# borgor/ripcurrents

Measured on AMD Instinct MI355X. Metric: frames/sec dense Farneback flow @1080p, higher is better.
Workload: dtype f32

## Files before the change

### ripcurrents_amd/csrc/flow_iter_kernels.hip

```cpp

#include <cstdlib>

#include "rc_device.h"

#define RC_ITER_BATCH 3
#define RC_RR_D 3

#ifdef RC_EXACT_BUILD
#define RC_FLOW_NS rc_flow_exact
#else
#define RC_FLOW_NS rc_flow_fast
#endif
namespace RC_FLOW_NS {

__device__ __forceinline__ float2 rc_flow_in(const RcIterArgs& a, const float2* fin, int gx, int gy) {
    if (a.in_mode == 0) return make_float2(0.f, 0.f);
    if (a.in_mode == 1) return fin[(size_t)gy * a.w + gx];
    float ax, ay;
    int sx = rc_src_x(gx, a.up_scale_x, a.fin_w, ax);
    int sx1 = min(sx + 1, a.fin_w - 1);
    int sy = rc_src_y(gy, a.up_scale_y, ay);
    int sy0 = rc_clampi(sy, 0, a.fin_h - 1), sy1 = rc_clampi(sy + 1, 0, a.fin_h - 1);
    const float2* S0 = fin + (size_t)sy0 * a.fin_w;
    const float2* S1 = fin + (size_t)sy1 * a.fin_w;
// ... 887 lines not shown
            p00[q] = S0[sx]; p01[q] = S0[sx1]; p10[q] = S1[sx]; p11[q] = S1[sx1];
        }
#pragma unroll
        for (int q = 0; q < NIT; q++) {
            float a0 = 1.f - ax, a1 = ax, b0 = 1.f - ay[q], b1 = ay[q];
            float r0x = p00[q].x * a0 + p01[q].x * a1, r1x = p10[q].x * a0 + p11[q].x * a1;
            float r0y = p00[q].y * a0 + p01[q].y * a1, r1y = p10[q].y * a0 + p11[q].y * a1;
            dx[q] = (r0x * b0 + r1x * b1) * a.up_mul;
            dy[q] = (r0y * b0 + r1y * b1) * a.up_mul;
        }
    }
}


__device__ __forceinline__ void rc_lds_barrier() { asm volatile("s_waitcnt lgkmcnt(0)\n\ts_barrier" ::: "memory"); }
__device__ __forceinline__ void rc_all_barrier() { asm volatile("s_waitcnt vmcnt(0) lgkmcnt(0)\n\ts_barrier" ::: "memory"); }

constexpr bool rc_recip_exact(int nt, int wp) {
    const unsigned r = (65536u + wp - 1) / wp;
    for (int t = 0; t < nt; t++)
        if ((int)((t * r) >> 16) != t / wp) return false;
    return true;
}

__device__ __forceinline__ void rc_glds16_s(const void* base, unsigned voff, uint32_t lds_wave_addr) {
    asm volatile("s_mov_b32 m0, %2\n\ts_nop 0\n\tglobal_load_lds_dwordx4 %0, %1" ::"v"(voff), "s"(base), "s"(lds_wave_addr) : "memory");
}
__device__ __forceinline__ void rc_glds4_s(const void* base, unsigned voff, uint32_t lds_wave_addr) {
    asm volatile("s_mov_b32 m0, %2\n\ts_nop 0\n\tglobal_load_lds_dword %0, %1" ::"v"(voff), "s"(base), "s"(lds_wave_addr) : "memory");
}

template <bool INTERIOR, int NT, int WP, int WN, int NWL>
__device__ __forceinline__ void rc_rrc_issue_window(const float4* __restrict__ RA1, const float* __restrict__ RB1,
                                                    uint32_t lds_a, uint32_t lds_b, int tid, int ox, int oy, int w, int h) {
    constexpr int QY = NT / WP, QX = NT % WP;
    const int wave_base = __builtin_amdgcn_readfirstlane(tid & ~63);
    static_assert(rc_recip_exact(NT, WP), "tid / WP by multiply and shift must be exact for every thread");
    int wy = (int)(__umul24((unsigned)tid, (65536u + WP - 1) / WP) >> 16), wx = tid - (int)__umul24((unsigned)wy, (unsigned)WP);
    int off = __mul24(oy + wy, w) + ox + wx;
#pragma unroll
    for (int q = 0; q < NWL; q++) {
        bool ok = (q + 1) * NT <= WN || tid + q * NT < WN;
        if (!INTERIOR) ok = ok && (unsigned)(ox + wx) < (unsigned)w && (unsigned)(oy + wy) < (unsigned)h;
        const unsigned p = ok ? (unsigned)off : 0u;
        if (q * NT + wave_base < WN) {
            rc_glds16_s(RA1, p << 4, lds_a + (uint32_t)(q * NT + wave_base) * 16u);
            rc_glds4_s(RB1, p << 2, lds_b + (uint32_t)(q * NT + wave_base) * 4u);
        }
        wx += QX; wy += QY; off += QY * w + QX;
        if (wx >= WP) { wx -= WP; wy += 1; off += w - WP; }
    }
}

template <bool INTERIOR, int NIT, int WW, int WH, int WP>
__device__ __forceinline__ void rc_rr_matrices(float (&m)[NIT][5], const float4 (&A0)[NIT], const float (&B0)[NIT],
                                               const float (&dx)[NIT], const float (&dy)[NIT], const float4* LA,
                                               const float* LB, int ox, int oy, const float4* __restrict__ RA1,
                                               const float* __restrict__ RB1, int gxo, const int (&gys)[NIT], int w, int h) {
    if constexpr (!INTERIOR) {
#pragma unroll
        for (int q = 0; q < NIT; q++) {
            RcGather g;
            rc_gather_window<WW, WH, WP>(g, LA, LB, ox, oy, RA1, RB1, gxo, gys[q], dx[q], dy[q], w, h);
            RcM5 v = rc_matrices_reg(A0[q], B0[q], g, dx[q], dy[q], gxo, gys[q], w, h, true);
            m[q][0] = v.m0; m[q][1] = v.m1; m[q][2] = v.m2; m[q][3] = v.m3; m[q][4] = v.m4;
        }
    } else {
        unsigned far = 0;
#pragma unroll
        for (int q = 0; q < NIT; q++) {
            RcGather g;
            const float fx = gxo + dx[q], fy = gys[q] + dy[q];
            const float flx = floorf(fx), fly = floorf(fy);
            const int x1 = (int)flx, y1 = (int)fly;
            g.fx = fx - flx;
            g.fy = fy - fly;
            g.inside = true;
            const int wx = x1 - ox, wy = y1 - oy;
            const bool in_win = (unsigned)wx < (unsigned)(WW - 1) && (unsigned)wy < (unsigned)(WH - 1);
            far |= in_win ? 0u : 1u << q;
            const unsigned i = in_win ? __umul24((unsigned)wy, (unsigned)WP) + (unsigned)wx : 0u;
            const float4* pa = (const float4*)((const char*)LA + (i << 4));
            const float* pb = (const float*)((const char*)LB + (i << 2));
            g.q00 = pa[0]; g.q01 = pa[1]; g.q10 = pa[WP]; g.q11 = pa[WP + 1];
            g.e00 = pb[0]; g.e01 = pb[1]; g.e10 = pb[WP]; g.e11 = pb[WP + 1];
            RcM5 v = rc_matrices_reg(A0[q], B0[q], g, dx[q], dy[q], gxo, gys[q], w, h, false);
            m[q][0] = v.m0; m[q][1] = v.m1; m[q][2] = v.m2; m[q][3] = v.m3; m[q][4] = v.m4;
        }
        if (__builtin_expect(far != 0, 0)) {
#pragma unroll
            for (int q = 0; q < NIT; q++) {
                if (far >> q & 1) {
                    RcGather g;
                    rc_gather_issue(g, RA1, RB1, gxo, gys[q], dx[q], dy[q], w, h);
                    RcM5 v = rc_matrices_reg(A0[q], B0[q], g, dx[q], dy[q], gxo, gys[q], w, h, false);
                    m[q][0] = v.m0; m[q][1] = v.m1; m[q][2] = v.m2; m[q][3] = v.m3; m[q][4] = v.m4;
                }
            }
        }
    }
}

template <bool INTERIOR, int IN_MODE, int GAUSS_, int NIT, int D, int MW, int NG>
__device__ __forceinline__ void rc_rrc_body(const RcIterArgs& a, const int zb, const int ze, float* smf, const uint32_t lds0, const int tx0, const int ty0) {
    constexpr int NT = NG * MW, MH = NG * NIT;
    constexpr int WW = MW + 2 * D, WH = MH + 2 * D, WP = WW, WN = WP * WH, NWL = (WN + NT - 1) / NT;
    constexpr int WNP = (WN + 63) & ~63;
    constexpr int MP = MW + 1, PLANE = MH * MP;
    static_assert(5 * PLANE <= 5 * WNP, "border-block M1 planes alias the R1 window");
    float4* LA = (float4*)smf;
    float* LB = smf + 4 * WNP;
    float* XR = LB + WNP;
    float* Ms = smf;
    const uint32_t lds_a = lds0, lds_b = lds0 + 16u * WNP;
    const int w = a.w, h = a.h;
    const int ox = tx0 - 2 - D, oy = ty0 - 2 - D;
#define RC_RRC_COORDS(tid_)                                                         \
    const int x = (tid_) & (MW - 1), grp = (tid_) / MW, ly0 = grp * NIT;            \
    const int px = tx0 - 2 + x;                                                     \
    const int gxo = INTERIOR ? px : rc_clampi(px, 0, w - 1);                        \
    int gys[NIT];                                                                   \
    _Pragma("unroll") for (int q = 0; q < NIT; q++)                                 \
        gys[q] = INTERIOR ? ty0 - 2 + ly0 + q : rc_clampi(ty0 - 2 + ly0 + q, 0, h - 1);

    float4 A0[NIT];
    float B0[NIT];
    float dx[NIT], dy[NIT];
    {
        const int tid = threadIdx.x;
        RC_RRC_COORDS(tid)
        const size_t s0 = (size_t)((a.slot0 + zb * a.zstep) % a.nslots) * a.R_slot_stride;
        const size_t s1 = (size_t)((a.slot1 + zb * a.zstep) % a.nslots) * a.R_slot_stride;
        rc_rrc_issue_window<INTERIOR, NT, WP, WN, NWL>(a.RA + s1, a.RB + s1, lds_a, lds_b, tid, ox, oy, w, h);
#pragma unroll
        for (int q = 0; q < NIT; q++) {
            const unsigned p0 = (unsigned)(gys[q] * w + gxo);
            A0[q] = (a.RA + s0)[p0];
            B0[q] = (a.RB + s0)[p0];
            rc_r0_prep(A0[q], B0[q]);
        }
        rc_rr_flow_in<IN_MODE, NIT, MW, MH, INTERIOR>(a, a.fin + (size_t)zb * a.fin_pair_stride, tx0, ty0, gxo, gys, dx, dy);
    }

    for (int z = zb; z < ze; z++) {
        const size_t s1 = (size_t)((a.slot1 + z * a.zstep) % a.nslots) * a.R_slot_stride;
        const float4* __restrict__ RA1 = a.RA + s1;
        const float* __restrict__ RB1 = a.RB + s1;
        const bool more = z + 1 < ze;
        int tid = threadIdx.x;
        asm volatile("" : "+v"(tid));
        RC_RRC_COORDS(tid)
        rc_all_barrier();

        float m[NIT][5];
        rc_rr_matrices<INTERIOR, NIT, WW, WH, WP>(m, A0, B0, dx, dy, LA, LB, ox, oy, RA1, RB1, gxo, gys, w, h);
        rc_rr_exchange<NIT, MW>(m, XR, grp, x);
        rc_lds_barrier();

        {
            float2 f1[NIT];
            rc_rr_flows<GAUSS_, NIT, MW, NG>(m, XR, grp, x, a.win, f1);
            float f1x[NIT], f1y[NIT];
#pragma unroll
            for (int q = 0; q < NIT; q++) { f1x[q] = f1[q].x; f1y[q] = f1[q].y; }
            rc_rr_matrices<INTERIOR, NIT, WW, WH, WP>(m, A0, B0, f1x, f1y, LA, LB, ox, oy, RA1, RB1, gxo, gys, w, h);
        }
        if (more) {
#pragma unroll
            for (int q = 0; q < NIT; q++) {
                const int i = (int)__umul24((unsigned)(gys[q] - oy), (unsigned)WP) + (gxo - ox);
                A0[q] = LA[i];
                B0[q] = LB[i];
                rc_r0_prep(A0[q], B0[q]);
            }
        }
        rc_lds_barrier();
        if constexpr (!INTERIOR) {
#pragma unroll
            for (int q = 0; q < NIT; q++)
#pragma unroll
                for (int c = 0; c < 5; c++) Ms[c * PLANE + (ly0 + q) * MP + x] = m[q][c];
            rc_lds_barrier();
#pragma unroll
            for (int q = 0; q < NIT; q++) {
                const int py = ty0 - 2 + ly0 + q;
                if ((unsigned)px >= (unsigned)w || (unsigned)py >= (unsigned)h) {
                    const int cx = gxo - (tx0 - 2), cy = gys[q] - (ty0 - 2);
#pragma unroll
                    for (int c = 0; c < 5; c++) m[q][c] = Ms[c * PLANE + cy * MP + cx];
                }
            }
        }
        rc_rr_exchange<NIT, MW>(m, XR, grp, x);
        rc_lds_barrier();

        if (more) {
            const size_t n1 = (size_t)((a.slot1 + (z + 1) * a.zstep) % a.nslots) * a.R_slot_stride;
            rc_rrc_issue_window<INTERIOR, NT, WP, WN, NWL>(a.RA + n1, a.RB + n1, lds_a, lds_b, tid, ox, oy, w, h);
        }

        {
            char* fout = a.fout + (size_t)z * a.fout_pair_stride;
            float2 f2[NIT];
            rc_rr_flows<GAUSS_, NIT, MW, NG>(m, XR, grp, x, a.win, f2);
            if (x >= 2 && x < MW - 2 && (INTERIOR || px < w)) {
                unsigned so = (unsigned)(ty0 - 2 + ly0) * (unsigned)a.fout_step + (unsigned)px * 8u;
#pragma unroll
                for (int q = 0; q < NIT; q++) {
                    const int ly = ly0 + q, py = ty0 - 2 + ly;
                    if (ly >= 2 && ly < MH - 2 && (INTERIOR || py < h)) *(float2*)(fout + so) = f2[q];
                    so += (unsigned)a.fout_step;
                }
            }
        }
        if (more) rc_rr_flow_in<IN_MODE, NIT, MW, MH, INTERIOR>(a, a.fin + (size_t)(z + 1) * a.fin_pair_stride, tx0, ty0, gxo, gys, dx, dy);
    }
#undef RC_RRC_COORDS
}

template <int IN_MODE, int GAUSS_, int NIT, int D, int MINB, int MW, int NG>
__global__ __launch_bounds__(NG * MW, MINB) void k_flow_iter2_rrc(RcIterArgs a, RcChainPlan cp) {
    constexpr int MH = NG * NIT, TW = MW - 4, TH = MH - 4;
    extern __shared__ __align__(16) float smf[];
    const int zb = cp.ngroups ? cp.start[blockIdx.y] : (int)blockIdx.y, ze = cp.ngroups ? cp.start[blockIdx.y + 1] : zb + 1;
    const int t = a.xcd_remap ? rc_xcd_remap(blockIdx.x, a.tiles_x * a.tiles_y) : (int)blockIdx.x;
    const int tx0 = (t % a.tiles_x) * TW, ty0 = (t / a.tiles_x) * TH;
    const bool interior = tx0 - 2 >= 5 && tx0 - 2 + MW <= a.w - 5 && ty0 - 2 >= 5 && ty0 - 2 + MH <= a.h - 5;
    const uint32_t lds0 = (uint32_t)(uintptr_t)(__attribute__((address_space(3))) void*)smf;
    if (interior) rc_rrc_body<true, IN_MODE, GAUSS_, NIT, D, MW, NG>(a, zb, ze, smf, lds0, tx0, ty0);
    else rc_rrc_body<false, IN_MODE, GAUSS_, NIT, D, MW, NG>(a, zb, ze, smf, lds0, tx0, ty0);
}

template <int IN_MODE, int G, int NIT, int D, int MINB, int MW = 32, int NG = 8>
static void launch_rrc_t(RcIterArgs a, const RcChainPlan& cp, int pairs, hipStream_t s) {
    constexpr int MH = NG * NIT, TW = MW - 4, TH = MH - 4;
    a.tw = TW; a.th = TH;
    a.tiles_x = (a.w + TW - 1) / TW; a.tiles_y = (a.h + TH - 1) / TH;
    constexpr int WN = (MW + 2 * D) * (MH + 2 * D), WNP = (WN + 63) & ~63;
    const size_t lds = sizeof(float) * (5 * WNP + NG * 2 * 5 * MW);
    RC_ALLOW_LDS((k_flow_iter2_rrc<IN_MODE, G, NIT, D, MINB, MW, NG>), lds);
    hipLaunchKernelGGL((k_flow_iter2_rrc<IN_MODE, G, NIT, D, MINB, MW, NG>), dim3(a.tiles_x * a.tiles_y, cp.ngroups ? cp.ngroups : pairs, 1), dim3(NG * MW), lds, s, a, cp);
}

static void rc_chain_plan(const RcIterArgs& a, int pairs, long long tiles, RcChainPlan& cp) {
    cp.ngroups = 0;
    const bool chainable = a.chain > 1 && pairs > 1 && (a.slot0 + a.zstep) % a.nslots == a.slot1 % a.nslots;
    if (!chainable) return;
    int chain = a.chain;
    if (!(a.ablate & RC_ABL_FORCE_CHAIN))
        while (chain > 1 && tiles * pairs / chain < (a.chain_min_blocks > 0 ? a.chain_min_blocks : 4096)) chain >>= 1;
    if (chain <= 1) return;
    int n = 0, z = 0;
    cp.start[0] = 0;
    while (z < pairs) {
        int left = pairs - z, c = left > chain ? chain : (left + 1) / 2;
        if (n == RC_MAX_CHAIN_GROUPS - 1) c = left;
        z += c;
        cp.start[++n] = z;
    }
    cp.ngroups = n;
}

template <int IN_MODE, int G>
static void launch_w3x2(RcIterArgs a, int pairs, hipStream_t s) {
    const long long tiles = (long long)((a.w + 27) / 28) * ((a.h + 27) / 28), blocks = tiles * pairs;
    RcChainPlan cp;
    rc_chain_plan(a, pairs, tiles, cp);
    if (cp.ngroups) launch_rrc_t<IN_MODE, G, 4, RC_RR_D, 4>(a, cp, pairs, s);
    else if (blocks < 512) launch_rrc_t<IN_MODE, G, 2, 4, 6>(a, cp, pairs, s);
    else if (blocks < 1024) launch_rrc_t<IN_MODE, G, 3, 4, 5>(a, cp, pairs, s);
    else launch_rrc_t<IN_MODE, G, 4, RC_RR_D, 4>(a, cp, pairs, s);
}

int rc_flow_iter_can_fuse2(const RcIterArgs& a) { return a.win.m == 1 && a.solve && a.addr32; }

int rc_flow_iter2_r0_reads(const RcIterArgs& a, int pairs) {
    RcChainPlan cp;
    rc_chain_plan(a, pairs, (long long)((a.w + 27) / 28) * ((a.h + 27) / 28), cp);
    return cp.ngroups ? cp.ngroups : pairs;
}

int rc_flow_chain_groups(const RcIterArgs& a, int pairs, int* starts, int cap) {
    RcChainPlan cp;
    rc_chain_plan(a, pairs, (long long)((a.w + 27) / 28) * ((a.h + 27) / 28), cp);
    for (int i = 0; i <= cp.ngroups && i < cap; i++) starts[i] = cp.start[i];
    return cp.ngroups;
}

void rc_launch_flow_iter2(const RcIterArgs& a, int pairs, hipStream_t s) {
    const int g = a.win.gaussian ? 1 : 0;
// ... 76 lines not shown
```

### ripcurrents_amd/csrc/rc_common.h

```cpp
#pragma once

#include <hip/hip_runtime.h>
#include <limits.h>
#include <stdint.h>

#include "../../include/rcflow.h"
#include "rc_plan.h"

#define RC_FMA(a, b, c) __builtin_fmaf((a), (b), (c))

__device__ __forceinline__ int rc_cvt_i32_x86(float v) {
    return (v >= -2147483648.f && v < 2147483648.f) ? (int)v : (int)0x80000000;
}

__device__ __forceinline__ const float2* rc_row2(const float* base, size_t step, int y) {
    return (const float2*)((const char*)base + (size_t)y * step);
}

__device__ __forceinline__ bool rc_sample_flow(const float* flow, size_t step, int w, int h, float x, float y,
                                               float& dx, float& dy) {
    int xind = rc_cvt_i32_x86(floorf(x)), yind = rc_cvt_i32_x86(floorf(y));
    float xrem = x - xind, yrem = y - yind;
    if (xind < 1 || yind < 1 || xind + 2 > w || yind + 2 > h) return false;
    const float2* r0 = rc_row2(flow, step, yind) + xind;
// ... 36 lines not shown
    const float* kern;
};

struct RcPolyArgs {
    const float* I;
    size_t I_slot_stride;
    const uint8_t* src8;
    size_t src8_step, src8_frame_stride;
    float4* RA;
    float* RB;
    size_t R_slot_stride;
    int slot0, nslots, zstep;
    int w, h;
    int tile_h;
    int valu_vertical;
    RcPolyK pk;
    int npyr;
    RcPyrFused py[2];
};

enum RcAblate : int {
    RC_ABL_EXACT_PLAIN_SCANS = 2,
    RC_ABL_EXACT_FUSED_M = 16,
    RC_ABL_PYR_STAGED = 4096,
    RC_ABL_TILE_WINDOW = 65536,
    RC_ABL_FORCE_SWEEP = 8388608,
    RC_ABL_FORCE_CHAIN = 33554432,
};

struct RcIterArgs {
    const float4* RA;
    const float* RB;
    size_t R_slot_stride;
    int slot0, slot1, nslots, zstep;
    int w, h;
    int in_mode;
    const float2* fin;
    size_t fin_pair_stride;
    int fin_w, fin_h;
    double up_scale_x, up_scale_y;
    float up_mul;
    int up_exact2;
    char* fout;
    size_t fout_step;
    size_t fout_pair_stride;
    int tw, th;
    int tiles_x, tiles_y;
    int solve;
    int xcd_remap;
    int ablate;
    int addr32;
    int chain_min_blocks;
    int chain;
    RcWindow win;
};

#define RC_MAX_CHAIN_GROUPS 64
struct RcChainPlan {
    int ngroups;
    int start[RC_MAX_CHAIN_GROUPS + 1];
};

struct RcExactArgs {
    const float4* RA;
    const float* RB;
    size_t n;
    int slot0, slot1, nslots, zstep;
    int w, h;
    const float2* fin;
    size_t fin_pair_stride;
    int fin_w, fin_h;
    double up_scale_x, up_scale_y;
    float up_mul;
    float2* flow;
    float* M;
    void* V;
    void* G;
    char* out;
    size_t out_step, out_pair_stride;
    int plain_scans;
    int fused_matrices;
    RcWindow win;
};
void rc_launch_exact_polyexp(const RcPolyArgs& a, int frames, hipStream_t s);
void rc_launch_exact_flow_init(const RcExactArgs& a, int pairs, hipStream_t s);
void rc_launch_exact_matrices(const RcExactArgs& a, int pairs, hipStream_t s);
void rc_launch_exact_window_solve(const RcExactArgs& a, int pairs, hipStream_t s);
int rc_exact_iteration_fused_ok(const RcExactArgs& a);
void rc_launch_exact_iteration_fused(const RcExactArgs& a, int pairs, hipStream_t s);

#define RC_MAX_DEVICES 64
#define RC_ALLOW_LDS(fn, lds)                                                                             \
    do {                                                                                                  \
        static size_t rc_seen_[RC_MAX_DEVICES] = {0};                                                     \
        int rc_dev_ = 0;                                                                                  \
        (void)hipGetDevice(&rc_dev_);                                                                     \
        if (rc_dev_ >= 0 && rc_dev_ < RC_MAX_DEVICES && (size_t)(lds) > rc_seen_[rc_dev_]) {             \
            (void)hipFuncSetAttribute((const void*)(fn), hipFuncAttributeMaxDynamicSharedMemorySize, (int)(lds)); \
            rc_seen_[rc_dev_] = (size_t)(lds);                                                            \
        }                                                                                                 \
    } while (0)

void rc_launch_pyr(const RcPyrArgs& a, int frames, size_t lds, hipStream_t s);
void rc_launch_polyexp(const RcPolyArgs& a, int frames, hipStream_t s);
int rc_polyexp_pyr_ok(const RcPolyArgs& a);
int rc_pyr_pair_ok(const RcPyrArgs& a1, const RcPyrArgs& a2);
// ... 32 lines not shown
```

### ripcurrents_amd/csrc/rc_host.h

```cpp
#pragma once

#include <initializer_list>
#include <string>
#include <vector>

#include "rc_common.h"

struct RcBuf {
    void* p = nullptr;
    size_t bytes = 0;
};

struct RcPlan {
    bool valid = false;
    int w = 0, h = 0;
    rc_farneback_params prm{};
    int nlev = 0;
    RcLevel lv[RC_MAX_LEVELS];
    size_t kern_off[RC_MAX_LEVELS];
    RcPolyK pk;
    RcWindow win;
    int nslots = 0, chunk = 0;
    int exact_taps = 0;
    int exact = 0;
// ... 180 lines not shown
    int ts_streak = 0;
    bool in_ts_push = false;
    RcPlan plan;
    RcBuf kern;
    RcBuf I[RC_MAX_LEVELS], RA[RC_MAX_LEVELS], RB[RC_MAX_LEVELS];
    RcBuf FA[RC_MAX_LEVELS], FB[RC_MAX_LEVELS];
    RcBuf stage_u8, stage_flow, stage_f32[4];
    RcBuf exM, exV, exG;
    void* pin[2] = {nullptr, nullptr};
    size_t pin_bytes = 0;
    hipEvent_t pin_free[2] = {nullptr, nullptr};
    int pin_i = 0;
    int pin_acq = -1, pin_w = 0, pin_h = 0;
    int flow_w = 0, flow_h = 0;
    int flow_fresh = 0;
    RcBuf lk;
    RcBuf fit_ws;
    RcBuf area_tab;
    RcBuf seed, seed_tab;
    int primed = 0, cur_slot = 0;
    int batch_primed = 0, batch_cur = 0;
    RcGraphCache batch_graph;
    RcGraphCache loop_graph;
    int loop_fc = 0;
    RcAnalysis an;
    RcTimex tx;
    RcFrameStab fs;
    RcRipMap rm;
    RcTracers tr;
    RcRegions rg;
    RcTracks tk;
    RcMotion mt;
    RcPhaseCorr pc;
};

struct RcProfRec {
    int id;
    hipEvent_t e0, e1;
    double bytes;
    double model_bytes;
};

struct rc_ctx {
    int device = 0;
    int max_w = 0, max_h = 0, nstreams = 0;
    RcSlot* slots = nullptr;
    int chunk = 32;
    int exact_taps = 0;
    int exact = -1;
    int fuse_iters = 1;
    int chain_min_blocks = 0;
    int chain = 8;
    int xcd_remap = 1;
    int poly_tile_h = 32;
    int frame_overlap = 1;
    int merge_small = 1;
    int overlap = 0;
    int poly_mfma = 0;
    int hist_blocks = 0;
    int fuse_pyr = 1;
    int ablate = 0;
    void* comm = nullptr;
    int prof_on = 0;
    std::vector<RcProfRec> prof_pending;
    std::vector<hipEvent_t> ev_pool;
    std::vector<int> prof_launches;
    std::vector<double> prof_ms, prof_bytes, prof_model_bytes;
};

#define RC_BUCKET_TABLE(X) \
    X(RC_B_FARNEBACK, "farneback") X(RC_B_POLAR, "polar") X(RC_B_THRESHOLD, "threshold") X(RC_B_OVERLAY, "overlay") \
    X(RC_B_EROSION, "erosion") X(RC_B_CODEC, "codec") X(RC_B_STREAM, "stream")
#define RC_KIND_TABLE(X) \
    X(RC_K_PYR, "pyr_level", RC_B_FARNEBACK) \
    X(RC_K_POLY, "polyexp", RC_B_FARNEBACK) \
    X(RC_K_ITER, "flow_iter", RC_B_FARNEBACK) \
    X(RC_K_HIST, "polar_hist", RC_B_THRESHOLD) \
    X(RC_K_THRESH, "thresholds", RC_B_THRESHOLD) \
    X(RC_K_CLASSIFY, "classify_accumulate", RC_B_THRESHOLD) \
    X(RC_K_ADVECT_FIELD, "advect_field", RC_B_STREAM) \
    X(RC_K_ADVECT_POINTS, "advect_points", RC_B_STREAM) \
    X(RC_K_POSTOP, "flow_postop", RC_B_FARNEBACK) \
    X(RC_K_COLOR, "flow_color", RC_B_THRESHOLD) \
    X(RC_K_ITER2, "flow_iter_x2", RC_B_FARNEBACK) \
    X(RC_K_PREPROC, "frame_preproc", RC_B_FARNEBACK) \
    X(RC_K_EDGES, "create_edges", RC_B_EROSION) \
    X(RC_K_DISPLAY, "streamline_display", RC_B_STREAM) \
    X(RC_K_HSV2BGR, "hsv_to_bgr", RC_B_THRESHOLD) \
    X(RC_K_OVERLAY, "create_output", RC_B_OVERLAY) \
    X(RC_K_FLOW_SEED, "flow_area_init", RC_B_FARNEBACK) \
    X(RC_K_TIMEX, "timex", RC_B_OVERLAY)  \
    X(RC_K_COLOR_U8, "frame_color", RC_B_OVERLAY)  \
    X(RC_K_FRAMESTAB, "framestab", RC_B_FARNEBACK)  \
    X(RC_K_RIPMAP, "ripmap", RC_B_FARNEBACK)  \
    X(RC_K_TRACKSTAB, "trackstab", RC_B_FARNEBACK)  \
    X(RC_K_TRACERS, "tracers", RC_B_STREAM)  \
    X(RC_K_REGIONS, "regions", RC_B_THRESHOLD)  \
    X(RC_K_TRACKS, "tracks", RC_B_THRESHOLD)  \
    X(RC_K_MOTION, "motion", RC_B_FARNEBACK)
#define RC_ROW_ID(id, ...) id,
enum { RC_BUCKET_TABLE(RC_ROW_ID) RC_B_BUCKETS };
enum { RC_KIND_TABLE(RC_ROW_ID) RC_K_KINDS };
enum { RC_K_LISTED = RC_K_MOTION };
static_assert(RC_K_LISTED == 25, "the rows before RC_K_MOTION keep their ids");
static_assert(RC_B_BUCKETS == RC_PROFILE_BUCKETS, "include/rcflow.h promises RC_PROFILE_BUCKETS buckets");

// ... 110 lines not shown
```

### ripcurrents_amd/csrc/rcflow_api.hip

```cpp

#include <cfloat>
#include <cmath>
#include <cstdarg>
#include <cstdio>
#include <cstring>

#include "rc_host.h"

static thread_local char g_err[512] = "";
void rc_set_error(const char* fmt, ...) {
    va_list ap;
    va_start(ap, fmt);
    vsnprintf(g_err, sizeof(g_err), fmt, ap);
    va_end(ap);
}
extern "C" const char* rcflow_last_error(void) { return g_err; }
extern "C" int rcflow_abi_version(void) { return RCFLOW_ABI_VERSION; }

int rc_buf_ensure(RcBuf& b, size_t bytes) {
    if (b.bytes >= bytes && b.p) return RC_OK;
    if (b.p) (void)hipFree(b.p);
    b.p = nullptr;
    b.bytes = 0;
    if (bytes == 0) return RC_OK;
// ... 276 lines not shown
    if (!s || !s->plan.valid || level < 0 || level >= s->plan.nlev || !d_flow) return RC_EINVAL;
    *d_flow = (float*)(which ? s->FB[level].p : s->FA[level].p);
    if (w) *w = s->plan.lv[level].w;
    if (h) *h = s->plan.lv[level].h;
    return *d_flow ? RC_OK : RC_ESTATE;
}

extern "C" int rcflow_debug_plan_poly(int n, double sigma, int exact_taps, float* g, float* xg, float* xxg, double* ig, int* n_eff,
                                      double* kdc) {
    if (n < 1 || n > RC_MAX_POLY_N || !(sigma >= 0) || !g || !xg || !xxg || !ig || !n_eff || !kdc) return RC_EINVAL;
    RcPolyK pk;
    const int rc = rc_plan_prepare_poly(n, sigma, exact_taps, pk);
    if (rc) return rc;
    memcpy(g, pk.g, (n + 1) * sizeof(float));
    memcpy(xg, pk.xg, (n + 1) * sizeof(float));
    memcpy(xxg, pk.xxg, (n + 1) * sizeof(float));
    ig[0] = pk.ig11; ig[1] = pk.ig03; ig[2] = pk.ig33; ig[3] = pk.ig55;
    *n_eff = pk.n_eff;
    *kdc = pk.kdc;
    return RC_OK;
}
extern "C" int rcflow_debug_plan_pyr_kernel(int ksize, double sigma, float* taps) {
    if (ksize < 1 || ksize > 1023 || !(sigma >= 0) || !taps) return RC_EINVAL;
    rc_plan_gaussian_kernel(ksize, sigma, taps);
    return RC_OK;
}
extern "C" int rcflow_debug_kind(int id, const char** name, const char** bucket) {
    if (id < 0 || id >= RC_K_LISTED || !name || !bucket) return RC_EINVAL;
    *name = kKindNames[id];
    *bucket = kBucketNames[kBucketOfKind[id]];
    return RC_OK;
}

extern "C" int rcflow_set_option(rc_ctx* ctx, const char* name, int value) {
    if (!ctx || !name) return RC_EINVAL;
    if (!strcmp(name, "chunk")) {
        if (value < 1 || value > 64) return RC_EINVAL;
        ctx->chunk = value;
    } else if (!strcmp(name, "exact_taps")) {
        ctx->exact_taps = value ? 1 : 0;
    } else if (!strcmp(name, "exact")) {
        if (value < -1 || value > 1) return RC_EINVAL;
        ctx->exact = value;
    } else if (!strcmp(name, "fuse_iters")) {
        ctx->fuse_iters = value ? 1 : 0;
    } else if (!strcmp(name, "chain")) {
        if (value < 1 || value > 64) return RC_EINVAL;
        ctx->chain = value;
    } else if (!strcmp(name, "chain_min_blocks")) {
        if (value < 0) return RC_EINVAL;
        ctx->chain_min_blocks = value;
    } else if (!strcmp(name, "xcd_remap")) {
        ctx->xcd_remap = value ? 1 : 0;
    } else if (!strcmp(name, "hist_blocks")) {
        if (value < 0 || value > 65535) return RC_EINVAL;
        ctx->hist_blocks = value;
    } else if (!strcmp(name, "overlap")) {
        ctx->overlap = value ? 1 : 0;
    } else if (!strcmp(name, "frame_overlap")) {
        if (value < 0 || value > 2) return RC_EINVAL;
        ctx->frame_overlap = value;
    } else if (!strcmp(name, "merge_small")) {
        ctx->merge_small = value ? 1 : 0;
    } else if (!strcmp(name, "poly_mfma")) {
        ctx->poly_mfma = value ? 1 : 0;
    } else if (!strcmp(name, "poly_tile_h")) {
        if (value != 32 && value != 48) return RC_EINVAL;
        ctx->poly_tile_h = value;
    } else if (!strcmp(name, "fuse_pyr")) {
        ctx->fuse_pyr = value != 0;
    } else if (!strcmp(name, "ablate")) {
        ctx->ablate = value;
    } else {
        rc_set_error("unknown option %s", name);
        return RC_EINVAL;
    }
    for (int i = 0; i < ctx->nstreams; i++) ctx->slots[i].plan.valid = false;
    return RC_OK;
}

extern "C" int rcflow_level_geometry(int w, int h, double pyr_scale, int levels, int k, int* wk, int* hk) {
    if (w <= 0 || h <= 0 || !(pyr_scale > 0 && pyr_scale < 1) || levels < 0 || k < 0) return RC_EINVAL;
    RcLevel L;
    rc_plan_level_geom(w, h, pyr_scale, k, L);
    if (wk) *wk = L.w;
    if (hk) *hk = L.h;
    return rc_plan_crop_levels(w, h, pyr_scale, levels);
}

static int ensure_plan(rc_ctx* ctx, RcSlot& s, int w, int h, const rc_farneback_params* p, int chunk, int nslots = 0) {
    if (nslots <= 0) nslots = chunk + 1;
    if (w <= 0 || h <= 0 || !rc_plan_params_valid(p)) {
        rc_set_error("invalid Farneback arguments (w=%d h=%d)", w, h);
        return RC_EINVAL;
    }
    if (w > ctx->max_w || h > ctx->max_h) {
        rc_set_error("frame %dx%d exceeds the context's %dx%d", w, h, ctx->max_w, ctx->max_h);
        return RC_ESIZE;
    }
    RcPlan& pl = s.plan;
    const rc_farneback_params& q = pl.prm;
    const bool same_prm = q.pyr_scale == p->pyr_scale && q.levels == p->levels && q.winsize == p->winsize &&
                          q.iterations == p->iterations && q.poly_n == p->poly_n && q.poly_sigma == p->poly_sigma &&
                          q.flags == p->flags;
    const int exact = ctx->exact >= 0 ? ctx->exact
                                      : (p->winsize / 2 == 0 || ((p->flags & RC_FARNEBACK_GAUSSIAN) && p->winsize / 2 <= 2));
    if (pl.valid && pl.w == w && pl.h == h && same_prm && pl.chunk == chunk &&
        pl.nslots == nslots && pl.exact_taps == ctx->exact_taps && pl.exact == exact)
        return RC_OK;
    rc_graph_drop(s.batch_graph);
    rc_graph_drop(s.loop_graph);
    RC_HIP(hipStreamSynchronize(s.cur));
    if (s.aux) RC_HIP(hipStreamSynchronize(s.aux));
    pl.valid = false;
    pl.w = w; pl.h = h; pl.chunk = chunk; pl.nslots = nslots;
    memset(&pl.prm, 0, sizeof(pl.prm));
    pl.prm.pyr_scale = p->pyr_scale; pl.prm.levels = p->levels; pl.prm.winsize = p->winsize;
    pl.prm.iterations = p->iterations; pl.prm.poly_n = p->poly_n; pl.prm.poly_sigma = p->poly_sigma;
    pl.prm.flags = p->flags;
    pl.exact_taps = ctx->exact_taps;
    pl.exact = exact;
    int L = rc_plan_crop_levels(w, h, p->pyr_scale, p->levels);
    pl.nlev = L + 1;
    size_t kern_total = 0;
    for (int k = 0; k <= L; k++) {
        rc_plan_level_geom(w, h, p->pyr_scale, k, pl.lv[k]);
        if (pl.lv[k].ksize > 1023) { rc_set_error("pyramid blur too wide"); return RC_EINVAL; }
        rc_plan_pick_pyr_tile(pl.lv[k], w, h);
        pl.kern_off[k] = kern_total;
        kern_total += (pl.lv[k].ksize + 3) & ~3;
    }
// ... 181 lines not shown
            a.fin = seeded; a.fin_pair_stride = a.n; a.fin_w = L.w; a.fin_h = L.h;
            a.up_scale_x = a.up_scale_y = 1.; a.up_mul = 1.f;
        }
        const double nb = (double)pairs * a.n;
        { RcProfScope ps(ctx, s.cur, RC_K_ITER, k, 8. * nb + (coarse ? 8. * pairs * cw * ch : seeded ? 8. * nb : 0.));
          rc_launch_exact_flow_init(a, pairs, s.cur); }
        for (int i = 0; i < iters; i++) {
            if (k == 0 && i == iters - 1) { a.out = (char*)d_out; a.out_step = out_step; a.out_pair_stride = out_pair_stride; }
            if (rc_exact_iteration_fused_ok(a)) {
                RcProfScope ps(ctx, s.cur, RC_K_ITER, k, 136. * nb);
                rc_launch_exact_iteration_fused(a, pairs, s.cur);
                continue;
            }
            { RcProfScope ps(ctx, s.cur, RC_K_ITER, k, 68. * nb); rc_launch_exact_matrices(a, pairs, s.cur); }
            { RcProfScope ps(ctx, s.cur, RC_K_ITER, k, (pl.win.gaussian ? 68. : 108.) * nb);
              rc_launch_exact_window_solve(a, pairs, s.cur); }
        }
        if (k == 0 && iters == 0)
            for (int z = 0; z < pairs; z++)
                RC_HIP(hipMemcpy2DAsync((char*)d_out + (size_t)z * out_pair_stride, out_step, a.flow + (size_t)z * a.n,
                                        (size_t)L.w * 8, (size_t)L.w * 8, (size_t)L.h, hipMemcpyDeviceToDevice, s.cur));
        coarse = a.flow;
        cw = L.w; ch = L.h;
    }
    RC_HIP(hipGetLastError());
    return RC_OK;
}

static int compute_flows(rc_ctx* ctx, RcSlot& s, int pairs, int slot0, float* d_out, size_t out_pair_stride,
                         size_t out_step, int slot1 = -1, int zstep = 1, const RcSeed* seed = nullptr) {
    if (!s.in_ts_push) s.ts_streak = 0;
    if (s.plan.exact && !s.plan.win.gaussian)
        return compute_flows_exact(ctx, s, pairs, slot0, d_out, out_pair_stride, out_step, slot1, zstep, seed);
    const bool exact = s.plan.exact != 0;
    RcPlan& pl = s.plan;
    const int iters = pl.prm.iterations;
    const float2* seeded = nullptr;
    if (seed) { int rc = launch_seed(ctx, s, pairs, *seed, &seeded); if (rc) return rc; }
    const float2* coarse = nullptr;
    int cw = 0, ch = 0;
    for (int k = pl.nlev - 1; k >= 0; k--) {
        const RcLevel& L = pl.lv[k];
        size_t n = (size_t)L.w * L.h;
        RcIterArgs a;
        memset(&a, 0, sizeof(a));
        a.RA = (const float4*)s.RA[k].p; a.RB = (const float*)s.RB[k].p; a.R_slot_stride = n;
        a.slot0 = slot0; a.slot1 = slot1 >= 0 ? slot1 : (slot0 + 1) % pl.nslots; a.nslots = pl.nslots; a.zstep = zstep;
        a.w = L.w; a.h = L.h;
        a.win = pl.win;
        a.xcd_remap = ctx->xcd_remap;
        a.ablate = ctx->ablate;
        a.chain = ctx->chain;
        a.chain_min_blocks = ctx->chain_min_blocks;
        const float2* cur_in = nullptr;
        int passes = iters > 0 ? iters : 1;
        int nout = 0;
        for (int i = 0; i < passes;) {
            double in_bytes;
            if (i == 0) {
                if (!coarse && seeded) { a.in_mode = 1; a.fin = seeded; a.fin_pair_stride = n; in_bytes = 8. * n; }
                else if (!coarse) { a.in_mode = 0; a.fin = nullptr; in_bytes = 0; }
                else {
                    a.in_mode = 2; a.fin = coarse; a.fin_pair_stride = (size_t)cw * ch;
                    a.fin_w = cw; a.fin_h = ch;
                    a.up_scale_x = 1. / ((double)L.w / cw);
                    a.up_scale_y = 1. / ((double)L.h / ch);
                    a.up_mul = (float)(1. / pl.prm.pyr_scale);
                    a.up_exact2 = (L.w == 2 * cw && L.h == 2 * ch) ? 1 : 0;
                    in_bytes = 8. * cw * ch;
                }
            } else {
                a.in_mode = 1; a.fin = cur_in; a.fin_pair_stride = n; in_bytes = 8. * n;
            }
            a.solve = iters > 0 ? 1 : 0;
            a.addr32 = n * 16 < (1ull << 32) && (size_t)L.h * (k == 0 ? (out_step > (size_t)L.w * 8 ? out_step : (size_t)L.w * 8) : (size_t)L.w * 8) < (1ull << 32);
            int fuse = (passes - i >= 2 && ctx->fuse_iters && rc_flow_fast::rc_flow_iter_can_fuse2(a)) ? 2 : 1;
            bool last = (i + fuse == passes);
            if (last && k == 0) {
                a.fout = (char*)d_out; a.fout_step = out_step; a.fout_pair_stride = out_pair_stride;
            } else {
                float2* dst = (float2*)((nout & 1) ? s.FB[k].p : s.FA[k].p);
                nout++;
                a.fout = (char*)dst; a.fout_step = (size_t)L.w * 8; a.fout_pair_stride = n * 8;
                cur_in = dst;
            }
            {
                double model = 0;
                if (i == 0) model += 60. * n + (coarse ? 8. * cw * ch : 0.);
                for (int j = i; j < i + fuse; j++) model += (j == passes - 1) ? 28. * n : 80. * n;
                const int r0 = fuse != 2 ? pairs : exact ? rc_flow_exact::rc_flow_iter2_r0_reads(a, pairs) : rc_flow_fast::rc_flow_iter2_r0_reads(a, pairs);
                RcProfScope ps(ctx, s.cur, fuse == 2 ? RC_K_ITER2 : RC_K_ITER, k,
                               (a.solve ? 20. * n * (pairs + r0) : 0.) + (double)pairs * (in_bytes + 8. * n), (double)pairs * model);
                if (exact) {
                    if (fuse == 2) rc_flow_exact::rc_launch_flow_iter2(a, pairs, s.cur);
                    else rc_flow_exact::rc_launch_flow_iter(a, pairs, s.cur);
                } else {
                    if (fuse == 2) rc_flow_fast::rc_launch_flow_iter2(a, pairs, s.cur);
                    else rc_flow_fast::rc_launch_flow_iter(a, pairs, s.cur);
                }
            }
            i += fuse;
        }
        coarse = cur_in;
        cw = L.w; ch = L.h;
    }
    RC_HIP(hipGetLastError());
// ... 362 lines not shown
    }
    cleanup();
    return rc;
}

void rc_graph_drop(RcGraphCache& g) {
    for (int i = 0; i < 2; i++) {
        if (g.exec[i]) (void)hipGraphExecDestroy((hipGraphExec_t)g.exec[i]);
        g.exec[i] = nullptr;
        g.eager[i] = 0;
    }
}

enum { RC_GRAPH_EAGER, RC_GRAPH_CAPTURE, RC_GRAPH_REPLAY };
static int graph_state(const RcGraphCache& g, int parity, const void* key, size_t key_bytes, bool allowed) {
    if (!allowed || memcmp(key, g.key[parity], key_bytes)) return RC_GRAPH_EAGER;
    return g.exec[parity] ? RC_GRAPH_REPLAY : g.eager[parity] ? RC_GRAPH_CAPTURE : RC_GRAPH_EAGER;
}

template <class Key, class Issue>
static int rc_graph_step(RcGraphCache& g, int parity, const Key& key, bool allowed, hipStream_t cap, hipStream_t run, Issue issue) {
    static_assert(sizeof(Key) <= sizeof(g.key[0]), "RcGraphCache::key too small");
    int rc;
    switch (graph_state(g, parity, &key, sizeof(key), allowed)) {
    case RC_GRAPH_REPLAY:
        RC_HIP(hipGraphLaunch((hipGraphExec_t)g.exec[parity], run));
        return RC_OK;
    case RC_GRAPH_CAPTURE: {
        hipGraph_t graph = nullptr;
        RC_HIP(hipStreamBeginCapture(cap, hipStreamCaptureModeRelaxed));
        rc = issue(cap);
        hipError_t e = hipStreamEndCapture(cap, &graph);
        if (rc) { if (graph) (void)hipGraphDestroy(graph); return rc; }
        if (e != hipSuccess || !graph) { rc_set_error("hipStreamEndCapture failed: %s", hipGetErrorString(e)); return RC_EHIP; }
        hipGraphExec_t exec = nullptr;
        e = hipGraphInstantiate(&exec, graph, nullptr, nullptr, 0);
        (void)hipGraphDestroy(graph);
        if (e != hipSuccess) { rc_set_error("hipGraphInstantiate failed: %s", hipGetErrorString(e)); return RC_EHIP; }
        g.exec[parity] = exec;
        RC_HIP(hipGraphLaunch(exec, run));
        return RC_OK;
    }
    default:
        if (g.exec[parity]) { (void)hipGraphExecDestroy((hipGraphExec_t)g.exec[parity]); g.exec[parity] = nullptr; }
        if ((rc = issue(run))) return rc;
        memcpy(g.key[parity], &key, sizeof(key));
        g.eager[parity] = 1;
        return RC_OK;
    }
}

struct RcLoopKey {
    rc_frame_loop loop;
    int w, h, pin, ring, ablate, chain;
    int seeded;
    void* hip_stream;
    void* d_frame; void* pin_host; void* d_flow;
};

static int loop_analysis(rc_ctx* ctx, RcSlot& s, int stream, const rc_frame_loop& L, int w, int h) {
    const size_t fs = (size_t)w * 8;
    float* d_flow = (float*)s.stage_flow.p;
    int rc;
    if ((rc = rc_loop_counter(ctx, s, false, 0))) return rc;
    if ((rc = rcflow_advect_field_dev(ctx, stream, d_flow, fs, w, h, L.dt, L.iterations, -1.f))) return rc;
    if (L.nseeds > 0 && (rc = rcflow_advect_points_dev(ctx, stream, L.d_seeds, L.nseeds, d_flow, fs, w, h, L.seed_dt, L.seed_iterations,
                                                       L.seed_upper, L.seed_variant, nullptr))) return rc;
    if ((rc = rcflow_histogram_dev(ctx, stream, d_flow, fs, w, h))) return rc;
    if ((rc = rcflow_thresholds_dev(ctx, stream))) return rc;
    if ((rc = rc_classify_accumulate(ctx, stream, d_flow, fs, w, h, -1, L.MID, L.LOWER, nullptr, 0, nullptr, 0, nullptr, 0,
                                     L.d_outmask, L.mask_step))) return rc;
    if (L.d_edges && (rc = rcflow_create_edges_dev(ctx, stream, L.d_outmask, L.mask_step, w, h, L.d_edges, L.edges_step))) return rc;
    return RC_OK;
}

static int loop_launches(rc_ctx* ctx, RcSlot& s, int stream, const rc_frame_loop& L, int pin, int w, int h, bool seeded) {
    const size_t fb = (size_t)w * h, fs = (size_t)w * 8;
    uint8_t* d_frame = (uint8_t*)s.stage_u8.p + (size_t)pin * fb;
    float* d_flow = (float*)s.stage_flow.p;
    const int cur = s.cur_slot, nxt = cur ^ 1;
    RC_HIP(hipMemcpyAsync(d_frame, s.pin[pin], fb, hipMemcpyHostToDevice, s.cur));
    int rc;
    if ((rc = expand_frames(ctx, s, d_frame, 0, w, 1, nxt))) return rc;
    const RcSeed seed = {d_flow, fs, 0};
    if ((rc = compute_flows(ctx, s, 1, cur, d_flow, 0, fs, nxt, 1, seeded ? &seed : nullptr))) return rc;
    return loop_analysis(ctx, s, stream, L, w, h);
}

extern "C" int rcflow_frame_loop_step(rc_ctx* ctx, int stream, const rc_farneback_params* p, const rc_frame_loop* loop) {
    RcSlot* s = rc_slot(ctx, stream);
    if (!s || !p || !loop) { if (s) rc_set_error("null argument"); return RC_EINVAL; }
    if (s->pin_acq < 0 || s->pin_acq != s->pin_i) { rc_set_error("no frame buffer acquired (rcflow_frame_buffer_acquire) since the last push"); return RC_ESTATE; }
    if (loop->nseeds < 0 || (loop->nseeds && !loop->d_seeds) || (loop->d_edges && !loop->d_outmask) || loop->iterations < 0) {
        rc_set_error("bad frame-loop configuration");
        return RC_EINVAL;
    }
    RC_HIP(hipSetDevice(ctx->device));
    const int w = s->pin_w, h = s->pin_h, pin = s->pin_acq;
    int rc;
    if (s->primed && s->an.w == w && s->an.h == h && (rc = rc_hist_book(*s, w, h, false))) return rc;
    if (!loop->use_graph) {
        if ((rc = rc_analysis_ensure(ctx, *s, w, h))) return rc;
        rc = push_staged_frame(ctx, s, pin, w, h, p);
        if (rc < 0) return rc;
        if (rc == 1) {
            s->loop_fc = 0;
            if ((rc = rc_loop_counter(ctx, *s, true, 0))) return rc;
            return 1;
        }
        if ((rc = loop_analysis(ctx, *s, stream, *loop, w, h))) return rc;
        s->loop_fc++;
        return RC_OK;
    }
    rc = ensure_plan(ctx, *s, w, h, p, 1, 2);
    if (rc) return rc;
    s->batch_primed = 0;
    if ((rc = rc_analysis_ensure(ctx, *s, w, h))) return rc;
    const size_t fb = (size_t)w * h;
    if (!s->primed) {
        rc_graph_drop(s->loop_graph);
        uint8_t* d_frame = (uint8_t*)s->stage_u8.p + (size_t)pin * fb;
        RC_HIP(hipMemcpyAsync(d_frame, s->pin[pin], fb, hipMemcpyHostToDevice, s->cur));
        RC_HIP(hipEventRecord(s->pin_free[pin], s->cur));
        if ((rc = expand_frames(ctx, *s, d_frame, 0, w, 1, 0))) return rc;
        s->loop_fc = 0;
        if ((rc = rc_loop_counter(ctx, *s, true, 0))) return rc;
        s->primed = 1; s->cur_slot = 0;
        s->pin_i = pin ^ 1; s->pin_acq = -1;
        s->flow_w = s->flow_h = 0;
        s->flow_fresh = 0;
        return 1;
    }
    const int cur = s->cur_slot;
    if (cur > 1) { rc_set_error("the slot's ring is not the frame loop's: call rcflow_stream_reset first"); return RC_ESTATE; }
    RcLoopKey key;
    memset(&key, 0, sizeof(key));
    key.loop = *loop;
    key.w = w; key.h = h; key.pin = pin; key.ring = cur; key.ablate = ctx->ablate; key.chain = ctx->chain;
    const bool seeded = (p->flags & RC_FARNEBACK_USE_INITIAL_FLOW) && s->flow_fresh && s->flow_w == w && s->flow_h == h;
    key.seeded = seeded;
    key.hip_stream = (void*)s->cur;
    key.d_frame = (uint8_t*)s->stage_u8.p + (size_t)pin * fb; key.pin_host = s->pin[pin]; key.d_flow = s->stage_flow.p;
    const bool graph_ok = !ctx->prof_on && s->cur != nullptr;
    const int state = graph_state(s->loop_graph, cur, &key, sizeof(key), graph_ok);
    if (state != RC_GRAPH_EAGER && (rc = rc_hist_book(*s, w, h, state == RC_GRAPH_REPLAY))) return rc;
    if ((rc = rc_graph_step(s->loop_graph, cur, key, graph_ok, s->cur, s->cur,
                            [&](hipStream_t) { return loop_launches(ctx, *s, stream, *loop, pin, w, h, seeded); })))
        return rc;
    if (state == RC_GRAPH_REPLAY) s->ts_streak = 0;
    RC_HIP(hipEventRecord(s->pin_free[pin], s->cur));
    s->cur_slot = cur ^ 1;
    s->pin_i = pin ^ 1; s->pin_acq = -1;
    s->flow_w = w; s->flow_h = h;
    s->flow_fresh = 1;
    s->loop_fc++;
    return RC_OK;
}

struct RcBatchKey {
    const void* frames; size_t frame_stride, step;
    void* flows; size_t flow_frame_stride, flow_step;
    void* hip_stream;
};

static int batch_launches(rc_ctx* ctx, RcSlot& s, const uint8_t* d_frames, size_t frame_stride, size_t step, int S,
                          float* d_flows, size_t flow_frame_stride, size_t flow_step, int cur) {
    int rc = expand_frames(ctx, s, d_frames, frame_stride, step, S, cur ^ 1, 2);
    if (rc) return rc;
    const RcSeed seed = {d_flows, flow_step, flow_frame_stride};
    const bool use_seed = (s.plan.prm.flags & RC_FARNEBACK_USE_INITIAL_FLOW) != 0;
    return compute_flows(ctx, s, S, cur, d_flows, flow_frame_stride, flow_step, cur ^ 1, 2, use_seed ? &seed : nullptr);
}

extern "C" int rcflow_push_batch_dev(rc_ctx* ctx, int stream, const uint8_t* d_frames, size_t frame_stride, size_t step,
                                     int nstreams, int w, int h, float* d_flows, size_t flow_frame_stride,
                                     size_t flow_step, const rc_farneback_params* p, int use_graph) {
    RcSlot* s = rc_slot(ctx, stream);
    if (!s || !d_frames || nstreams < 1 || nstreams > 4096) { if (s) rc_set_error("bad batch arguments"); return RC_EINVAL; }
    if (step < (size_t)w || (nstreams > 1 && frame_stride < step * (size_t)(h - 1) + w)) {
        rc_set_error("batch strides smaller than a frame");
        return RC_EINVAL;
    }
    RC_HIP(hipSetDevice(ctx->device));
    int rc = ensure_plan(ctx, *s, w, h, p, nstreams, 2 * nstreams);
    if (rc) return rc;
    s->primed = 0;
    if (!s->batch_primed) {
        rc_graph_drop(s->batch_graph);
        if ((rc = expand_frames(ctx, *s, d_frames, frame_stride, step, nstreams, 0, 2))) return rc;
        s->batch_primed = 1;
        s->batch_cur = 0;
// ... 150 lines not shown
```

Measured before the change: 19930.

## Shift LDS R1 window to follow the tile's incoming flow hint

For interior tiles with an incoming flow field, the kernel reads the flow at the tile centre, rounds it to integer pixels, and offsets the staged R1 window by that displacement so the gathered neighbourhood sits where the warped samples will actually land. The goal is to cut fallback global reads when displacement pushes samples outside the window. When the tile's own pixels fall outside the shifted window, the next iteration's R0 values come from global memory and are prepped lazily. It adds per-iteration hint loads, a scalar shift computation and a new option, and it depends on one flow sample being representative of the whole tile.

```diff
diff --git a/ripcurrents_amd/csrc/flow_iter_kernels.hip b/ripcurrents_amd/csrc/flow_iter_kernels.hip
--- a/ripcurrents_amd/csrc/flow_iter_kernels.hip
+++ b/ripcurrents_amd/csrc/flow_iter_kernels.hip
@@ -963,6 +963,35 @@
     }
 }
 
+__device__ __forceinline__ int rc_hint_round(int bits, int mulq8) {
+    const int sh = 142 - ((bits >> 23) & 255);
+    const unsigned m = ((unsigned)bits & 0x7fffffu) | 0x800000u;
+    const unsigned q8 = sh > 24 ? 0u : sh < 5 ? 0x7ffffu : m >> sh;
+    const int r = (int)((q8 * (unsigned)mulq8 + 32768u) >> 16);
+    return bits < 0 ? -r : r;
+}
+template <int IN_MODE, int MW, int MH>
+__device__ __forceinline__ float2 rc_rrc_hint(const RcIterArgs& a, const float2* __restrict__ fin, int tx0, int ty0) {
+    if constexpr (IN_MODE == 0) {
+        return make_float2(0.f, 0.f);
+    } else {
+        const int cx = tx0 - 2 + MW / 2, cy = ty0 - 2 + MH / 2;
+        if constexpr (IN_MODE == 1) {
+            return fin[(unsigned)(cy * a.w + cx)];
+        } else {
+            const int ux = min((int)__umulhi((unsigned)cx, a.hint_mx), a.fin_w - 1);
+            const int uy = min((int)__umulhi((unsigned)cy, a.hint_my), a.fin_h - 1);
+            return fin[(unsigned)(uy * a.fin_w + ux)];
+        }
+    }
+}
+template <int WW, int WH>
+__device__ __forceinline__ void rc_rrc_shift(const RcIterArgs& a, float2 hint, int ox, int oy, int w, int h, int& wox, int& woy) {
+    const int bx = __builtin_amdgcn_readfirstlane(__float_as_int(hint.x)), by = __builtin_amdgcn_readfirstlane(__float_as_int(hint.y));
+    wox = max(min(ox + rc_hint_round(bx, a.hint_mulq8), w - WW), 0);
+    woy = max(min(oy + rc_hint_round(by, a.hint_mulq8), h - WH), 0);
+}
+
 template <bool INTERIOR, int NIT, int WW, int WH, int WP>
 __device__ __forceinline__ void rc_rr_matrices(float (&m)[NIT][5], const float4 (&A0)[NIT], const float (&B0)[NIT],
                                                const float (&dx)[NIT], const float (&dy)[NIT], const float4* LA,
@@ -1026,6 +1055,8 @@
     const uint32_t lds_a = lds0, lds_b = lds0 + 16u * WNP;
     const int w = a.w, h = a.h;
     const int ox = tx0 - 2 - D, oy = ty0 - 2 - D;
+    const bool follow = INTERIOR && IN_MODE != 0 && a.window_follow;
+    int wox = ox, woy = oy;
 #define RC_RRC_COORDS(tid_)                                                         \
     const int x = (tid_) & (MW - 1), grp = (tid_) / MW, ly0 = grp * NIT;            \
     const int px = tx0 - 2 + x;                                                     \
@@ -1042,7 +1073,8 @@
         RC_RRC_COORDS(tid)
         const size_t s0 = (size_t)((a.slot0 + zb * a.zstep) % a.nslots) * a.R_slot_stride;
         const size_t s1 = (size_t)((a.slot1 + zb * a.zstep) % a.nslots) * a.R_slot_stride;
-        rc_rrc_issue_window<INTERIOR, NT, WP, WN, NWL>(a.RA + s1, a.RB + s1, lds_a, lds_b, tid, ox, oy, w, h);
+        if (follow) rc_rrc_shift<WW, WH>(a, rc_rrc_hint<IN_MODE, MW, MH>(a, a.fin + (size_t)zb * a.fin_pair_stride, tx0, ty0), ox, oy, w, h, wox, woy);
+        rc_rrc_issue_window<INTERIOR, NT, WP, WN, NWL>(a.RA + s1, a.RB + s1, lds_a, lds_b, tid, wox, woy, w, h);
 #pragma unroll
         for (int q = 0; q < NIT; q++) {
             const unsigned p0 = (unsigned)(gys[q] * w + gxo);
@@ -1053,6 +1085,7 @@
         rc_rr_flow_in<IN_MODE, NIT, MW, MH, INTERIOR>(a, a.fin + (size_t)zb * a.fin_pair_stride, tx0, ty0, gxo, gys, dx, dy);
     }
 
+    bool r0_raw = false;
     for (int z = zb; z < ze; z++) {
         const size_t s1 = (size_t)((a.slot1 + z * a.zstep) % a.nslots) * a.R_slot_stride;
         const float4* __restrict__ RA1 = a.RA + s1;
@@ -1062,9 +1095,16 @@
         asm volatile("" : "+v"(tid));
         RC_RRC_COORDS(tid)
         rc_all_barrier();
+        if (r0_raw) {
+#pragma unroll
+            for (int q = 0; q < NIT; q++) rc_r0_prep(A0[q], B0[q]);
+            r0_raw = false;
+        }
+        float2 hint = make_float2(0.f, 0.f);
+        if constexpr (INTERIOR && IN_MODE != 0) hint = rc_rrc_hint<IN_MODE, MW, MH>(a, a.fin + (size_t)(more ? z + 1 : z) * a.fin_pair_stride, tx0, ty0);
 
         float m[NIT][5];
-        rc_rr_matrices<INTERIOR, NIT, WW, WH, WP>(m, A0, B0, dx, dy, LA, LB, ox, oy, RA1, RB1, gxo, gys, w, h);
+        rc_rr_matrices<INTERIOR, NIT, WW, WH, WP>(m, A0, B0, dx, dy, LA, LB, wox, woy, RA1, RB1, gxo, gys, w, h);
         rc_rr_exchange<NIT, MW>(m, XR, grp, x);
         rc_lds_barrier();
 
@@ -1074,15 +1114,27 @@
             float f1x[NIT], f1y[NIT];
 #pragma unroll
             for (int q = 0; q < NIT; q++) { f1x[q] = f1[q].x; f1y[q] = f1[q].y; }
-            rc_rr_matrices<INTERIOR, NIT, WW, WH, WP>(m, A0, B0, f1x, f1y, LA, LB, ox, oy, RA1, RB1, gxo, gys, w, h);
+            rc_rr_matrices<INTERIOR, NIT, WW, WH, WP>(m, A0, B0, f1x, f1y, LA, LB, wox, woy, RA1, RB1, gxo, gys, w, h);
         }
         if (more) {
-#pragma unroll
-            for (int q = 0; q < NIT; q++) {
-                const int i = (int)__umul24((unsigned)(gys[q] - oy), (unsigned)WP) + (gxo - ox);
-                A0[q] = LA[i];
-                B0[q] = LB[i];
-                rc_r0_prep(A0[q], B0[q]);
+            const bool own_in_window = (unsigned)(ox + D - wox) <= (unsigned)(WW - MW) && (unsigned)(oy + D - woy) <= (unsigned)(WH - MH);
+            if (own_in_window) {
+#pragma unroll
+                for (int q = 0; q < NIT; q++) {
+                    const int i = (int)__umul24((unsigned)(gys[q] - woy), (unsigned)WP) + (gxo - wox);
+                    A0[q] = LA[i];
+                    B0[q] = LB[i];
+                    rc_r0_prep(A0[q], B0[q]);
+                }
+            } else {
+                unsigned p0 = (unsigned)(gys[0] * w + gxo);
+#pragma unroll
+                for (int q = 0; q < NIT; q++) {
+                    A0[q] = *(const float4*)((const char*)RA1 + (p0 << 4));
+                    B0[q] = *(const float*)((const char*)RB1 + (p0 << 2));
+                    p0 += (unsigned)w;
+                }
+                r0_raw = true;
             }
         }
         rc_lds_barrier();
@@ -1107,7 +1159,8 @@
 
         if (more) {
             const size_t n1 = (size_t)((a.slot1 + (z + 1) * a.zstep) % a.nslots) * a.R_slot_stride;
-            rc_rrc_issue_window<INTERIOR, NT, WP, WN, NWL>(a.RA + n1, a.RB + n1, lds_a, lds_b, tid, ox, oy, w, h);
+            if (follow) rc_rrc_shift<WW, WH>(a, hint, ox, oy, w, h, wox, woy);
+            rc_rrc_issue_window<INTERIOR, NT, WP, WN, NWL>(a.RA + n1, a.RB + n1, lds_a, lds_b, tid, wox, woy, w, h);
         }
 
         {
@@ -1147,6 +1200,14 @@
     constexpr int MH = NG * NIT, TW = MW - 4, TH = MH - 4;
     a.tw = TW; a.th = TH;
     a.tiles_x = (a.w + TW - 1) / TW; a.tiles_y = (a.h + TH - 1) / TH;
+    a.hint_mulq8 = 256;
+    if (a.in_mode == 2) {
+        const unsigned long long mx = ((unsigned long long)a.fin_w << 32) / a.w, my = ((unsigned long long)a.fin_h << 32) / a.h;
+        a.hint_mx = (unsigned)(mx < 0xffffffffull ? mx : 0xffffffffull);
+        a.hint_my = (unsigned)(my < 0xffffffffull ? my : 0xffffffffull);
+        const float m = a.up_mul * 256.f;
+        a.hint_mulq8 = m >= 4095.f ? 4095 : m >= 0.f ? (int)(m + 0.5f) : 0;
+    }
     constexpr int WN = (MW + 2 * D) * (MH + 2 * D), WNP = (WN + 63) & ~63;
     const size_t lds = sizeof(float) * (5 * WNP + NG * 2 * 5 * MW);
     RC_ALLOW_LDS((k_flow_iter2_rrc<IN_MODE, G, NIT, D, MINB, MW, NG>), lds);
diff --git a/ripcurrents_amd/csrc/rc_common.h b/ripcurrents_amd/csrc/rc_common.h
--- a/ripcurrents_amd/csrc/rc_common.h
+++ b/ripcurrents_amd/csrc/rc_common.h
@@ -112,6 +112,9 @@
     int addr32;
     int chain_min_blocks;
     int chain;
+    int window_follow;
+    unsigned hint_mx, hint_my;
+    int hint_mulq8;
     RcWindow win;
 };
 
diff --git a/ripcurrents_amd/csrc/rc_host.h b/ripcurrents_amd/csrc/rc_host.h
--- a/ripcurrents_amd/csrc/rc_host.h
+++ b/ripcurrents_amd/csrc/rc_host.h
@@ -256,6 +256,7 @@
     int chain_min_blocks = 0;
     int chain = 8;
     int xcd_remap = 1;
+    int window_follow = 1;
     int poly_tile_h = 32;
     int frame_overlap = 1;
     int merge_small = 1;
diff --git a/ripcurrents_amd/csrc/rcflow_api.hip b/ripcurrents_amd/csrc/rcflow_api.hip
--- a/ripcurrents_amd/csrc/rcflow_api.hip
+++ b/ripcurrents_amd/csrc/rcflow_api.hip
@@ -352,6 +352,9 @@
         ctx->chain_min_blocks = value;
     } else if (!strcmp(name, "xcd_remap")) {
         ctx->xcd_remap = value ? 1 : 0;
+    } else if (!strcmp(name, "window_follow")) {
+        if (value != 0 && value != 1) return RC_EINVAL;
+        ctx->window_follow = value;
     } else if (!strcmp(name, "hist_blocks")) {
         if (value < 0 || value > 65535) return RC_EINVAL;
         ctx->hist_blocks = value;
@@ -377,6 +380,11 @@
     }
     for (int i = 0; i < ctx->nstreams; i++) ctx->slots[i].plan.valid = false;
     return RC_OK;
+}
+
+extern "C" int rcflow_debug_option_check(const char* name, int value) {
+    rc_ctx c;
+    return rcflow_set_option(&c, name, value);
 }
 
 extern "C" int rcflow_level_geometry(int w, int h, double pyr_scale, int levels, int k, int* wk, int* hk) {
@@ -664,6 +672,7 @@
         a.ablate = ctx->ablate;
         a.chain = ctx->chain;
         a.chain_min_blocks = ctx->chain_min_blocks;
+        a.window_follow = ctx->window_follow;
         const float2* cur_in = nullptr;
         int passes = iters > 0 ? iters : 1;
         int nout = 0;
@@ -1132,7 +1141,7 @@
 
 struct RcLoopKey {
     rc_frame_loop loop;
-    int w, h, pin, ring, ablate, chain;
+    int w, h, pin, ring, ablate, chain, window_follow;
     int seeded;
     void* hip_stream;
     void* d_frame; void* pin_host; void* d_flow;
@@ -1217,6 +1226,7 @@
     memset(&key, 0, sizeof(key));
     key.loop = *loop;
     key.w = w; key.h = h; key.pin = pin; key.ring = cur; key.ablate = ctx->ablate; key.chain = ctx->chain;
+    key.window_follow = ctx->window_follow;
     const bool seeded = (p->flags & RC_FARNEBACK_USE_INITIAL_FLOW) && s->flow_fresh && s->flow_w == w && s->flow_h == h;
     key.seeded = seeded;
     key.hip_stream = (void*)s->cur;
```

After: 20030 (median of 6 runs). Within noise of the previous version (+0.5%).
